# jhuldr/BrainFM

Measured on AMD Instinct MI355X. Metric: voxels/sec whole-volume multi-task inference, 256^3 tiled, higher is better.
Workload: dtype f16x3-split (fp32-grade); 1 GPU; 256^3 volume, reference tiling win160/stride80 -> 27 tiles, UNet3D f64 x6 levels, 9 heads (69 ch), fused tail + deformed atlas + on-device stitch of 17 keys; stitched_keys=17, mfma_passes=3, submission=hipGraph replay per tile shape, parallelism=tiles sharded over 1 rank(s), gather to rank 0, tiles_in_flight_per_gpu=2

## Files before the change

brainfm_amd/_lib.py:

```python
import ctypes as C
import os

_HERE = os.path.dirname(os.path.abspath(__file__))
LIB_PATH = os.path.join(_HERE, "libbrainfm_hip.so")

ERR = {0: "BFM_OK", -1: "BFM_E_ARG", -2: "BFM_E_SHAPE", -3: "BFM_E_WORKSPACE", -4: "BFM_E_LAUNCH"}

ROLE_PLAIN, ROLE_CT, ROLE_BIAS_LOG, ROLE_SEG, ROLE_DIST, ROLE_SR, ROLE_PATHOL = range(7)
(EW_EXP, EW_AFFINE, EW_CLAMP, EW_CLAMP_MIN, EW_GAMMA, EW_SIGMOID, EW_DIV, EW_NONZERO, EW_SUB_DIV, EW_GE,
 EW_NAN_TO_NUM) = range(11)
(EW_ADD, EW_MUL, EW_MUL_EXP, EW_AXPY_CLAMP0, EW_AXPY, EW_DIV2, EW_ZERO_WHERE_ZERO) = range(7)


class BfmError(RuntimeError):
    pass


class Upsample(C.Structure):
    _fields_ = [("d", C.c_int), ("h", C.c_int), ("w", C.c_int),
                ("mapD", C.c_void_p), ("mapH", C.c_void_p), ("mapW", C.c_void_p),
                ("repD", C.c_void_p), ("repH", C.c_void_p), ("repW", C.c_void_p)]


CLASS_STATS_BLOCKS = 1024
# ... 44 lines not shown
    _fields_ = [("V", C.c_void_p), ("n", C.c_int64)]


class GatherJob(C.Structure):
    _fields_ = [("src", C.c_void_p), ("out", C.c_void_p), ("mean", C.c_float), ("scale", C.c_float), ("pre", C.c_int),
                ("default_max", C.c_int), ("post_div", C.c_float), ("clamp", C.c_int), ("clamp_lo", C.c_float),
                ("clamp_hi", C.c_float), ("sign", C.c_float), ("want_minmax", C.c_int)]


_P = C.c_void_p
_I = C.c_int
_F = C.c_float
_L = C.c_int64
_Z = C.c_size_t
_UP = C.POINTER(Upsample)

SIGNATURES = {
    "bfm_version": (C.c_char_p, []),
    "bfm_gn_stats_workspace": (_Z, [_I, _I, _I, _I, _I, _UP]),
    "bfm_gn_stats": (_I, [_P, _I, _P, _I, _I, _I, _I, _UP, _P, _P, _I, _F, _P, _P, _P, _P, _Z, _P]),
    "bfm_pack_conv_weights_direct": (_I, [_P, _I, _I, _P, _P]),
    "bfm_pack_conv_weights_mfma_bytes": (_Z, [_I, _I]),
    "bfm_pack_conv_weights_mfma": (_I, [_P, _I, _I, _F, _P, C.POINTER(_I), _P]),
    "bfm_pack_conv_weights_mfma16_bytes": (_Z, [_I, _I]),
    "bfm_pack_conv_weights_mfma16": (_I, [_P, _I, _I, _F, _P, C.POINTER(_I), _P]),
    "bfm_conv3x3x3_direct": (_I, [_P, _I, _P, _I, _I, _I, _I, _UP, _P, _P, _P, _I, _F, _P, _P]),
    "bfm_pack_conv_weights_upfold_bytes": (C.c_size_t, [_I, _I, _I]),
    "bfm_pack_conv_weights_upfold": (_I, [_P, _I, _I, _I, _F, _I, _P, _P, _P]),
    "bfm_conv3x3x3_upfold": (_I, [_P, _I, _I, _I, _I, _P, _P, _P, _I, _P, _I, _I, _I, _P, _P]),
    "bfm_conv3x3x3_upfold_workspace": (_Z, [_I, _I, _I, _I, _I]),
    "bfm_conv3x3x3_upfold_ex": (_I, [_P, _I, _I, _I, _I, _P, _P, _P, _I, _P, _I, _I, _I, _P, _P, _Z, _P]),
    "bfm_conv3x3x3_upfold_batch_workspace": (_Z, [_I, _I, _I, _I, _I, _I]),
    "bfm_conv3x3x3_upfold_batch": (_I, [_P, _I, _I, _I, _I, _I, _P, _P, _P, _I, _P, _I, _I, _I, _P, _P, _Z, _I, _P]),
    "bfm_moment_rows_bytes": (_Z, [_I, _I]),
    "bfm_conv3x3x3_mfma_rows": (_I, [_I, _I, _I, _I, _I, C.POINTER(_I)]),
    "bfm_conv3x3x3_mfma_ex": (_I, [_P, _I, _P, _I, _I, _I, _I, _UP, _P, _P, _P, _I, _P, _I, _I, _F, _I,
                                   C.POINTER(_I), _P, _P, _Z, _P, _P]),
    "bfm_conv3x3x3_mfma_batch_workspace": (_Z, [_I, _I, _I, _I, _I, _I, _I]),
    "bfm_conv3x3x3_mfma_batch": (_I, [_P, _I, _P, _I, _I, _I, _I, _I, _UP, _P, _P, _P, _I, _P, _I, _I, _F, _I,
                                      C.POINTER(_I), _P, _P, _Z, _P, _I, _P]),
    "bfm_gn_stats_batch_workspace": (_Z, [_I, _I, _I, _I, _I, _I, _UP]),
    "bfm_gn_stats_batch": (_I, [_P, _I, _P, _I, _I, _I, _I, _I, _UP, _P, _P, _I, _F, _P, _P, _P, _P, _Z, _P]),
    "bfm_gn_stats_rows_batch": (_I, [_P, _I, _I, _P, _I, _I, C.c_double, _L, _I, _P, _P, _I, _F, _P, _P, _P, _P]),
    "bfm_conv3x3x3_stem_rows": (_I, [_I, _I, _I]),
    "bfm_conv3x3x3_stem_ex": (_I, [_P, _I, _I, _I, _P, _P, _P, _P, _I, _F, _P, _P, _P]),
    "bfm_conv3x3x3_stem_mc_ex": (_I, [_P, _I, _I, _I, _I, _P, _P, _P, _P, _I, _F, _P, _P, _P]),
    "bfm_gn_stats_rows_workspace": (_Z, [_I, _I, _I, _I]),
    "bfm_gn_stats_rows": (_I, [_P, _I, _I, _P, _I, _I, C.c_double, _L, _P, _P, _I, _F, _P, _P, _P, _P, _Z, _P, _P]),
    "bfm_gn_stats_rows_sliced": (_I, [_P, _I, _I, _I, _I, _P, _I, _I, _I, _I, C.c_double, _L, _P, _P, _I, _F, _P, _P, _P, _P, _Z,
                                      _P, _P]),
    "bfm_gn_stats_rows_train": (_I, [_P, _I, _I, _P, _I, _I, C.c_double, _L, _P, _P, _I, _F, _P, _P, _P, _P, _P, _P, _Z, _P, _P]),
    "bfm_crop3d": (_I, [_P, _I, _I, _I, _I, _I, _I, _I, _I, _I, _P, _P]),
    "bfm_pack_conv_weights_wino4_bytes": (_Z, [_I, _I, _I]),
    "bfm_pack_conv_weights_wino4": (_I, [_P, _I, _I, _F, _I, _P, C.POINTER(_I), _P]),
    "bfm_conv3x3x3_wino4_rows": (_I, [_I, _I, _I, _I]),
    "bfm_conv3x3x3_wino4_box": (_I, [_I, _I, _I, _I, _P]),
    "bfm_conv3x3x3_wino4_masked_workspace": (_Z, [_I, _I, _I, _I]),
    "bfm_conv3x3x3_wino4_uniform_scratch": (_Z, [_I]),
    "bfm_conv3x3x3_wino4_uniform": (_I, [_P, _I, _I, _I, _I, _P, _P, _P, _I, _P, _I, _I, _F, _I, _I, _P, _P, _P, _P, _P]),
    "bfm_conv3x3x3_wino4": (_I, [_P, _I, _I, _I, _I, _P, _P, _P, _I, _P, _I, _I, _F, _I, _I, _P, _P, _P]),
    "bfm_conv3x3x3_wino4_batch": (_I, [_P, _I, _I, _I, _I, _I, _P, _P, _P, _I, _P, _I, _I, _F, _I, _I, _P, _P, _I, _P]),
    "bfm_conv3x3x3_wino4_masked": (_I, [_P, _I, _I, _I, _I, _P, _P, _P, _I, _P, _I, _I, _F, _I, _I, _P, _P, _P, _Z, _P]),
    "bfm_permute_flip3d": (_I, [_P, _I, _I, _I, C.POINTER(_I), C.POINTER(_I), _P, _P]),
    "bfm_bbox_nonzero": (_I, [_P, _I, _I, _I, _F, _P, _P]),
    "bfm_mean_lastdim": (_I, [_P, _L, _I, _P, _P]),
    "bfm_pack_conv_weights_wino_bytes": (_Z, [_I, _I, _I]),
# ... 229 lines not shown
```

brainfm_amd/engine.py:

```python
import ctypes as C
import os
from collections import OrderedDict, namedtuple

import numpy as np
import torch

from . import _lib as L

LABELS_LEFT = [0, 1, 2, 3, 4, 7, 8, 9, 10, 14, 15, 17, 31, 34, 36, 38, 40, 42]
LABELS_FULL = [0, 11, 12, 13, 16, 31, 32, 33, 34, 35, 36, 37, 38, 39, 40, 41, 42, 43, 44, 46,
               1, 2, 3, 4, 5, 6, 7, 8, 9, 10, 14, 15, 17, 47, 49, 51, 53, 55,
               18, 19, 20, 21, 22, 23, 24, 25, 26, 27, 28, 29, 30, 48, 50, 52, 54, 56]


def features_per_level(f_maps, num_levels):
    return [f_maps * 2 ** k for k in range(num_levels)]


def nearest_index_map(n_in, n_out):
    scale = np.float32(n_in) / np.float32(n_out)
    idx = np.floor(np.arange(n_out, dtype=np.float32) * scale).astype(np.int64)
    return np.minimum(idx, n_in - 1).astype(np.int32)


_TUNE_CHOICES = {}

_Variant = namedtuple("_Variant", "layout pack_bytes pack rows box dense masked_workspace masked uniform_scratch uniform",
                      defaults=(None,) * 7)
_MFMA = _Variant("mfma", "bfm_pack_conv_weights_mfma_bytes", "bfm_pack_conv_weights_mfma")
_CONV_VARIANTS = (
    _MFMA,
    _MFMA,
    _Variant("mfma16", "bfm_pack_conv_weights_mfma16_bytes", "bfm_pack_conv_weights_mfma16"),
    _Variant("wino", "bfm_pack_conv_weights_wino_bytes", "bfm_pack_conv_weights_wino", "bfm_conv3x3x3_wino_rows",
             "bfm_conv3x3x3_wino_box", "bfm_conv3x3x3_wino_ex", "bfm_conv3x3x3_wino_masked_workspace",
             "bfm_conv3x3x3_wino_masked", "bfm_conv3x3x3_wino_uniform_scratch", "bfm_conv3x3x3_wino_uniform"),
    _Variant("wino4", "bfm_pack_conv_weights_wino4_bytes", "bfm_pack_conv_weights_wino4", "bfm_conv3x3x3_wino4_rows",
             "bfm_conv3x3x3_wino4_box", "bfm_conv3x3x3_wino4", "bfm_conv3x3x3_wino4_masked_workspace",
             "bfm_conv3x3x3_wino4_masked", "bfm_conv3x3x3_wino4_uniform_scratch", "bfm_conv3x3x3_wino4_uniform"),
)
_VARIANT_OF = {v.layout: ver for ver, v in enumerate(_CONV_VARIANTS)}

TUNE_FILE = os.environ.get("BFM_CONV_TUNE_FILE") or os.path.join(os.path.dirname(os.path.abspath(__file__)),
                                                                  "conv_tune_gfx950.json")
_TUNE_TABLE = None
_ARCH = {}


def _tune_key_str(key):
    cin, cout, dims, two, acc = key[:5]
    return ",".join(str(int(v)) for v in (cin, cout) + tuple(dims) + (two, acc) + tuple(key[5:]))


def _arch_of(dev_index):
    if dev_index not in _ARCH:
# ... 45 lines not shown

TRAIN_F43 = os.environ.get("BFM_TRAIN_F43", "1") != "0"


class _Layer:
    __slots__ = ("name", "cin", "cout", "groups", "gamma", "beta", "kind", "wpacked", "wexp", "w_raw", "packs", "skip",
                 "used")

    def touch(self, layout):
        u = getattr(self, "used", None)
        if u is None:
            u = self.used = set()
        u.add(layout)


HEAD_SLOPE = 0.2


class _HeadLayer(_Layer):
    __slots__ = ("bias",)


class UNetEngine:
    prof = None
    lane = 0
    weights_epoch = 0
    pack_count = 0
    _ws_lanes = None
    _variants = None
    _f23_ids = None
    _same_box_cache = None
    _uf_cache = None
    _deep_ok = None
    _head_layers = None
    _unit_bound = None
    _no_heads = None
    dense_last = False
    tape = None
    grad_sink = None
    prof_reps = 1
    use_upfold = False
    upfold_min = 250
    fuse_stats = False

    def __init__(self, state_dict, in_channels=1, f_maps=64, num_levels=6, num_groups=8, unit_feat=True,
                 device="cuda", passes=3, eps=1e-5, slope=0.01):
        self.lib = L.load()
        self.device = torch.device(device)
        if self.device.type != "cuda":
            raise L.BfmError("UNetEngine needs a HIP device; the product path has no CPU fallback")
        self.fm = features_per_level(f_maps, num_levels) if isinstance(f_maps, int) else list(f_maps)
        self.in_channels = in_channels
        self.num_groups = num_groups
        self.unit_feat = bool(unit_feat)
        self.passes = int(passes)
        self.eps = float(eps)
        self.slope = float(slope)
        self._up_cache = {}
        self._ws_lanes = {}
        self._ws_retired = []
        self.lane = 0
        self._gn_tickets = {ln: torch.zeros(16, dtype=torch.int32, device=self.device) for ln in range(4)}
        self._uf_tickets = {ln: torch.zeros(1, dtype=torch.int32, device=self.device) for ln in range(4)}
        self.gn_one_launch = os.environ.get("BFM_GN_ONE_LAUNCH", "1") != "0"
        self._plan_cache = {}
        self._tuned = set()
# ... 143 lines not shown
                    jobs.append((ly, layout, absmax(ly.w_raw[:, ly.skip.cin:])))
                elif layout == "direct":
                    jobs.append((ly, layout, None))
                else:
                    if wm is None:
                        wm = absmax(ly.w_raw)
                    jobs.append((ly, layout, wm))
            ly.used = set()
            ly.wpacked, ly.kind = None, None
            if ly.skip is not None:
                ly.skip.w_raw.copy_(ly.w_raw[:, :ly.skip.cin])
                visit(ly.skip)

        for pair in self.enc + self.dec + [hidden]:
            for ly in pair:
                visit(ly)
        host = slots[:nslot[0]].cpu().tolist() if nslot[0] else []
        for ly, layout, m in jobs:
            wmax = host[m] if m is not None else None
            if layout == "upfold":
                self._make_upfold_pack(ly, ly.skip.cin, ly.cin - ly.skip.cin, wmax)
            else:
                self._make_pack(ly, layout, wmax)

    def _upsample_desc(self, lo, hi):
        key = (tuple(lo), tuple(hi))
        if key not in self._up_cache:
            maps = [nearest_index_map(lo[a], hi[a]) for a in range(3)]
            reps = [np.bincount(maps[a], minlength=lo[a]).astype(np.int32) for a in range(3)]
            dev = [torch.from_numpy(m).to(self.device) for m in maps + reps]
            up = L.Upsample(lo[0], lo[1], lo[2], *[t.data_ptr() for t in dev])
            self._up_cache[key] = (up, dev)
        return self._up_cache[key][0]

    def _workspace(self, nbytes):
        nbytes = max(int(nbytes), 256)
        if self._ws_lanes is None:
            self._ws_lanes, self._ws_retired = {}, []
        ws = self._ws_lanes.get(self.lane)
        if ws is None or ws.numel() < nbytes:
            if ws is not None:
                self._ws_retired.append(ws)
            ws = self._ws_lanes[self.lane] = torch.empty(int(nbytes * 1.25) + 1024, dtype=torch.uint8, device=self.device)
        return ws

    def _uf_ticket(self):
        t = self._uf_tickets
        if self.lane not in t:
            t[self.lane] = torch.zeros(1, dtype=torch.int32, device=self.device)
        return t[self.lane]

    def _gn_ticket(self):
        t = self._gn_tickets
        if self.lane not in t:
            t[self.lane] = torch.zeros(16, dtype=torch.int32, device=self.device)
        return t[self.lane]

    def _plan(self, cin, cout, dims, two_src=False, accum=False):
        key = (cin, cout, tuple(dims), bool(two_src), bool(accum))
        if key not in self._plan_cache:
            cfg = (C.c_int * 8)()
            L.check(self.lib.bfm_conv3x3x3_mfma_plan(cin, cout, dims[0], dims[1], dims[2], cfg), "mfma_plan")
            if two_src and cfg[6] in (3, 4):
                cfg[6] = 0
            self._plan_cache[key] = cfg
        return self._plan_cache[key]
# ... 438 lines not shown
        if fused is not None and out is None and self.tape is None:
            return fused
        if out is None:
            out = torch.empty((D // 2, H // 2, W // 2, c), dtype=torch.float32, device=self.device)
        rows = self._rows_buf(c, 1, self.lib.bfm_maxpool2_rows, c, D, H, W)
        L.check(self.lib.bfm_maxpool2_ex(L.ptr(X), c, D, H, W, L.ptr(out), L.ptr(rows[0]) if rows is not None else None,
                                         L.stream_ptr()), "maxpool2")
        if rows is not None:
            out._bfm_rows = rows
        if self.tape is not None:
            self.tape.append(dict(pool_in=X, pool_dims=tuple(dims)))
        return out, (D // 2, H // 2, W // 2)

    def maxpool_batch(self, X, dims):
        S, (D, H, W), c = X.shape[0], dims, X.shape[-1]
        out = torch.empty((S, D // 2, H // 2, W // 2, c), dtype=torch.float32, device=self.device)
        if c % 4 or self.tape is not None:
            for s_ in range(S):
                self.maxpool(X[s_], dims, out=out[s_])
            return out
        rows = self._rows_buf(c, S, self.lib.bfm_maxpool2_batch_rows, c, D, H, W)
        L.check(self.lib.bfm_maxpool2_batch(L.ptr(X), c, S, D, H, W, L.ptr(out), L.ptr(rows[0]) if rows is not None else None,
                                            L.stream_ptr()), "maxpool2_batch")
        if rows is not None:
            out._bfm_rows = rows
        return out

    deep_from = int(os.environ.get("BFM_DEEP_FROM", "3"))
    deep_batch = os.environ.get("BFM_DEEP_BATCH", "1") != "0"
    DEEP_VERS = (0, 2)
    DEEP_VERS_1SRC = (0, 2, 4)
    deep_upfold = os.environ.get("BFM_DEEP_UPFOLD", "1") != "0"
    deep_upfold_min = int(os.environ.get("BFM_DEEP_UPFOLD_MIN", "100"))
    mask_skip = os.environ.get("BFM_MASK_SKIP", "1") != "0"
    uniform_skip = os.environ.get("BFM_UNIFORM_SKIP", "1") != "0"

    deep_vox = int(os.environ.get("BFM_DEEP_VOX", "16000"))

    def _region_ok(self, df):
        if self._deep_ok is None:
            self._deep_ok = {}
        cache = self._deep_ok
        if df not in cache:
            ndeep = len(self.enc) - 1 - df
            layers = [ly for pair in self.enc[df:] + self.dec[:ndeep] for ly in pair]
            cache[df] = all(ly.cin % 16 == 0 and ly.cout % 64 == 0 for ly in layers) and \
                self.enc[df - 1][1].cout % 16 == 0
        return cache[df]

    def has_deep_region(self):
        if not (self.deep_batch and self.tape is None and not self.force_direct and len(self.fm) > self.deep_from >= 1):
            return False
        return self._region_ok(self.deep_from)

    def region_start(self, dims):
        df = self.deep_from
        while df - 1 >= 2:
            lv = [v >> (df - 1) for v in dims]
            if min(lv) < 1 or lv[0] * lv[1] * lv[2] > self.deep_vox or not self._region_ok(df - 1):
                break
            df -= 1
        return df

    def _batch_stats(self, ly, A, ca, B, cb, S, dims, lo_dims, upp, scale, shift, bound):
        D, H, W = dims
        st = L.stream_ptr()
        ra = getattr(A, "_bfm_rows", None) if self.fuse_stats else None
        rb = getattr(B, "_bfm_rows", None) if (self.fuse_stats and B is not None) else None
        exact2 = B is None or tuple(dims) == tuple(2 * v for v in lo_dims)
        if ra is not None and ra[1] <= 128 and (B is None or (rb is not None and exact2 and rb[1] <= 128)):
            L.check(self.lib.bfm_gn_stats_rows_batch(L.ptr(ra[0]), ra[1], ca, L.ptr(rb[0]) if rb is not None else None,
                                                     rb[1] if rb is not None else 0, cb, 8.0, D * H * W, S,
                                                     L.ptr(ly.gamma), L.ptr(ly.beta), ly.groups, self.eps, L.ptr(scale),
                                                     L.ptr(shift), L.ptr(bound), st), "gn_stats_rows_batch " + ly.name)
            return
        need = self.lib.bfm_gn_stats_batch_workspace(ca, cb, S, D, H, W, upp)
        ws = self._workspace(need)
        L.check(self.lib.bfm_gn_stats_batch(L.ptr(A), ca, L.ptr(B), cb, S, D, H, W, upp, L.ptr(ly.gamma), L.ptr(ly.beta),
                                            ly.groups, self.eps, L.ptr(scale), L.ptr(shift), L.ptr(bound), L.ptr(ws),
                                            ws.numel(), st), "gn_stats_batch " + ly.name)

    def batch_conv(self, ly, A, dims, B=None, lo_dims=None, stats=None):
        S = A.shape[0]
        D, H, W = dims
        ca = A.shape[-1]
        cb = 0 if B is None else B.shape[-1]
        assert ca + cb == ly.cin, (ly.name, ca, cb, ly.cin)
        if not self._mfma_ok(ly, ca, cb):
            raise L.BfmError("%s: the batched levels need channel counts that are multiples of 16 / 64" % ly.name)
        up = self._upsample_desc(lo_dims, dims) if B is not None else None
        upp = C.byref(up) if up is not None else None
        if stats is None:
            scale = torch.empty((S, ly.cin), dtype=torch.float32, device=self.device)
            shift = torch.empty((S, ly.cin), dtype=torch.float32, device=self.device)
            bound = torch.empty((S, ly.groups), dtype=torch.float32, device=self.device)
            self._batch_stats(ly, A, ca, B, cb, S, dims, lo_dims, upp, scale, shift, bound)
        else:
            scale, shift, bound = stats
        if (B is not None and self.use_upfold and self.deep_upfold and tuple(dims) == tuple(2 * v for v in lo_dims)
                and lo_dims[0] * lo_dims[1] * lo_dims[2] >= self.deep_upfold_min):
            return self._batch_conv_upfold(ly, A, dims, B, lo_dims, scale, shift, bound)
        key = (ly.cin, ly.cout, tuple(dims), B is not None, False, 1)
        vers = self.DEEP_VERS if B is not None else self.DEEP_VERS_1SRC
        cfg = self._batch_plan(key, vers)
        out = torch.empty((S, D, H, W, ly.cout), dtype=torch.float32, device=self.device)
        if key not in self._tuned:
            cfg = self._autotune(ly, key, lambda c: self._batch_launch(ly, c, A[0:1], B[0:1] if B is not None else None, upp, dims,
                                                                       scale[0:1], shift[0:1], bound[0:1], out[0:1]),
                                 vers=vers)
        self._pack(ly, True, cfg[6])
        rows = self._rows_for(ly.cin, ly.cout, dims, cfg, S)
        nv = D * H * W
        lo = 0 if B is None else lo_dims[0] * lo_dims[1] * lo_dims[2]
        self._bracket(lambda: self._batch_launch(ly, cfg, A, B, upp, dims, scale, shift, bound, out, rows),
                      lambda: (2.0 * 27 * ly.cin * ly.cout * nv * S,
                               4.0 * (S * (nv * ca + lo * cb + nv * ly.cout) + 27 * ly.cin * ly.cout),
                               self._tag(ly) + ("x%d" % S), ly.cin, ly.cout, dims, cfg))
        if rows is not None:
            out._bfm_rows = rows
        return out

    def _batch_plan(self, key, vers):
        if key not in self._plan_cache:
            cfg = (C.c_int * 8)()
            L.check(self.lib.bfm_conv3x3x3_mfma_plan(key[0], key[1], key[2][0], key[2][1], key[2][2], cfg), "mfma_plan")
            if cfg[6] not in vers:
                cfg[6] = 0
            if key[4]:
                cfg[7] = 1
            self._plan_cache[key] = cfg
        return self._plan_cache[key]
# ... 24 lines not shown
        st = L.stream_ptr()
        sk = self._skip_layer(ly, ca)
        if "upfold" not in ly.packs:
            self._make_upfold_pack(ly, ca, cb)
        ly.touch("upfold")
        wup, wexp_up = ly.packs["upfold"]
        sc_a, sh_a = scale[:, :ca], shift[:, :ca]
        sc_b, sh_b = scale[:, ca:], shift[:, ca:]
        aff = ca + cb
        out = torch.empty((S, D, H, W, ly.cout), dtype=torch.float32, device=self.device)
        key = (ca, ly.cout, tuple(dims), False, True, 1)
        cfg = self._batch_plan(key, self.DEEP_VERS_1SRC)
        if key not in self._tuned:
            cfg = self._autotune(sk, key, lambda c: self._batch_launch(sk, c, A[0:1], None, None, dims, sc_a[0:1], sh_a[0:1],
                                                                       bound[0:1], out[0:1], None, aff),
                                 vers=self.DEEP_VERS_1SRC)
        self._pack(sk, True, cfg[6])
        nv = D * H * W
        lo = lo_dims[0] * lo_dims[1] * lo_dims[2]
        wsu = self.lib.bfm_conv3x3x3_upfold_batch_workspace(cb, S, lo_dims[0], lo_dims[1], lo_dims[2], ly.cout)

        def _launch_up():
            ws = self._workspace(wsu)
            L.check(self.lib.bfm_conv3x3x3_upfold_batch(L.ptr(B), cb, S, lo_dims[0], lo_dims[1], lo_dims[2], L.ptr(sc_b),
                                                        L.ptr(sh_b), L.ptr(bound), ly.groups, L.ptr(wup), wexp_up,
                                                        ly.cout, self.passes, L.ptr(out), L.ptr(ws) if wsu else None,
                                                        ws.numel() if wsu else 0, aff, st), "conv_upfold_batch " + ly.name)
        self._bracket(_launch_up, lambda: (2.0 * 27 * cb * ly.cout * nv * S, 4.0 * (S * (lo * cb + nv * ly.cout)),
                                           self._tag(ly) + "x%dup" % S, cb, ly.cout, dims, (0,) * 8))
        rows = self._rows_for(ca, ly.cout, dims, cfg, S)
        self._bracket(lambda: self._batch_launch(sk, cfg, A, None, None, dims, sc_a, sh_a, bound, out, rows, aff),
                      lambda: (2.0 * 27 * ca * ly.cout * nv * S, 4.0 * S * (nv * ca + 2 * nv * ly.cout),
                               self._tag(ly) + "x%dsk" % S, ca, ly.cout, dims, cfg))
        if rows is not None:
            out._bfm_rows = rows
        return out

    def deep_region(self, tops, df=None):
        S = len(tops)
        df = self.deep_from if df is None else df
        dims0 = tuple(tops[0][1])
        assert all(tuple(d) == dims0 for _, d in tops)
        c0 = tops[0][0].shape[-1]
        d = tuple(v // 2 for v in dims0)
        if min(dims0) < 2:
            raise L.BfmError("volume too small for %d pooling levels" % (len(self.enc) - 1))
        l1, l2 = self.enc[df]
        P = torch.empty((S,) + d + (c0,), dtype=torch.float32, device=self.device)
        scale = torch.empty((S, l1.cin), dtype=torch.float32, device=self.device)
        shift = torch.empty((S, l1.cin), dtype=torch.float32, device=self.device)
        bound = torch.empty((S, l1.groups), dtype=torch.float32, device=self.device)
        for s_, (x, dd) in enumerate(tops):
            ps, _ = self.maxpool(x, dd, out=P[s_])
            self._gn_stats(l1, ps, c0, None, 0, d, None, None, scale[s_], shift[s_], bound[s_], 0)
        x = self.batch_conv(l1, P, d, stats=(scale, shift, bound))
        x = self.batch_conv(l2, x, d)
        skips = [(x, d)]
        for i in range(df + 1, len(self.enc)):
            l1, l2 = self.enc[i]
            if min(d) < 2:
                raise L.BfmError("volume too small for %d pooling levels" % (len(self.enc) - 1))
            d2 = tuple(v // 2 for v in d)
            P = self.maxpool_batch(x, d)
            d = d2
            x = self.batch_conv(l1, P, d)
            x = self.batch_conv(l2, x, d)
# ... 328 lines not shown
```

include/brainfm_hip.h:

```cpp
#ifndef BRAINFM_HIP_H
#define BRAINFM_HIP_H

#include <stddef.h>
#include <stdint.h>

#ifdef __cplusplus
extern "C" {
#endif

typedef void* bfm_stream_t;

#define BFM_OK 0
#define BFM_E_ARG (-1)
#define BFM_E_SHAPE (-2)
#define BFM_E_WORKSPACE (-3)
#define BFM_E_LAUNCH (-4)

typedef struct {
    int d, h, w;
    const int32_t* mapD; const int32_t* mapH; const int32_t* mapW;
    const int32_t* repD; const int32_t* repH; const int32_t* repW;
} bfm_upsample_t;

const char* bfm_version(void);
// ... 119 lines not shown
                        int flags, float* out, void* moment_rows , bfm_stream_t stream);
int bfm_conv3x3x3_wino4_batch(const float* A, int CA, int S, int D, int H, int W, const float* scale, const float* shift,
                              const float* bound, int G, const void* wpacked, int wexp, int Cout, float slope, int passes,
                              int flags, float* out, void* moment_rows, int affine_stride, bfm_stream_t stream);
size_t bfm_conv3x3x3_wino4_masked_workspace(int D, int H, int W, int passes);
size_t bfm_conv3x3x3_wino4_uniform_scratch(int Cout);
int bfm_conv3x3x3_wino4_uniform(const float* A, int CA, int D, int H, int W, const float* scale, const float* shift,
                                const float* bound, int G, const void* wpacked, int wexp, int Cout, float slope, int passes,
                                int flags, float* out, void* moment_rows, const unsigned char* uniform_flags, void* scratch,
                                bfm_stream_t stream);
int bfm_conv3x3x3_wino4_masked(const float* A, int CA, int D, int H, int W, const float* scale, const float* shift,
                               const float* bound, int G, const void* wpacked, int wexp, int Cout, float slope, int passes,
                               int flags, float* out, const float* mask_image, void* workspace, size_t workspace_bytes,
                               bfm_stream_t stream);

size_t bfm_conv3x3x3_mfma_workspace(int Cin, int Cout, int D, int H, int W, int splitk);
int bfm_conv3x3x3_mfma_plan(int Cin, int Cout, int D, int H, int W, int* cfg_out );

size_t bfm_pack_conv_weights_upfold_bytes(int CB, int Cout, int passes);
int bfm_pack_conv_weights_upfold(const float* w_oidhw , int CA, int CB, int Cout,
                                 float wmax_abs_host, int passes, void* wpacked, int* wexp_host, bfm_stream_t stream);
int bfm_conv3x3x3_upfold(const float* B, int CB, int d, int h, int w, const float* scale_b, const float* shift_b,
                         const float* bound, int G, const void* wpacked, int wexp, int Cout, int passes, float* out,
                         bfm_stream_t stream);
size_t bfm_conv3x3x3_upfold_workspace(int CB, int d, int h, int w, int Cout);
int bfm_conv3x3x3_upfold_ex(const float* B, int CB, int d, int h, int w, const float* scale_b, const float* shift_b,
                            const float* bound, int G, const void* wpacked, int wexp, int Cout, int passes, float* out,
                            void* workspace, size_t workspace_bytes, bfm_stream_t stream);
size_t bfm_conv3x3x3_upfold_batch_workspace(int CB, int S, int d, int h, int w, int Cout);
int bfm_conv3x3x3_upfold_batch(const float* B, int CB, int S, int d, int h, int w, const float* scale_b,
                               const float* shift_b, const float* bound, int G, const void* wpacked, int wexp, int Cout,
                               int passes, float* out, void* workspace, size_t workspace_bytes, int affine_stride,
                               bfm_stream_t stream);

int bfm_conv3x3x3_mfma(const float* A, int CA, const float* B, int CB, int D, int H, int W,
                       const bfm_upsample_t* up, const float* scale, const float* shift, const float* bound,
                       int G, const void* wpacked, int wexp, int Cout, float slope, int passes,
                       const int* cfg , float* out, void* workspace,
                       size_t workspace_bytes, bfm_stream_t stream);

int bfm_maxpool2(const float* in, int C, int D, int H, int W, float* out, bfm_stream_t stream);

enum {
    BFM_ROLE_PLAIN = 0,
    BFM_ROLE_CT = 1,
    BFM_ROLE_BIAS_LOG = 2,
    BFM_ROLE_SEG = 3,
    BFM_ROLE_DIST = 4,
    BFM_ROLE_SR = 5,
    BFM_ROLE_PATHOL = 6
};
typedef struct {
    int n_out;
    int c_feat;
    const float* head_w;
    const float* head_b;
    const int32_t* roles;
    const int32_t* out_slot;
    int seg_first, n_seg;
    const int32_t* seg_lut;
    int n_dist;
    int dist_first;
    float max_dist;
    int unit_feat;
    int slot_high_res;
    int slot_fake_cortical;
// ... 350 lines not shown
```

Baseline: 204.5 million voxels/s.

## Add per-tap GEMM conv path for tiny deep-level volumes

Adds a new convolution path for very small spatial volumes (at most 64 low-res voxels). It packs the normalized activations once into f16 hi/lo splits, runs one MFMA GEMM per kernel tap (optionally split-K across slabs) to fill the CUs, then gathers and sums the 27 tap partials through a precomputed row table. That table also folds in nearest upsampling and applies the activation and moment stats. This is meant to fix the poor occupancy of the regular conv kernels on the deepest UNet levels, at the cost of extra workspace traffic for the partials and an additional launch.

```diff
diff --git a/brainfm_amd/_lib.py b/brainfm_amd/_lib.py
--- a/brainfm_amd/_lib.py
+++ b/brainfm_amd/_lib.py
@@ -100,6 +100,10 @@
     "bfm_conv3x3x3_upfold_ex": (_I, [_P, _I, _I, _I, _I, _P, _P, _P, _I, _P, _I, _I, _I, _P, _P, _Z, _P]),
     "bfm_conv3x3x3_upfold_batch_workspace": (_Z, [_I, _I, _I, _I, _I, _I]),
     "bfm_conv3x3x3_upfold_batch": (_I, [_P, _I, _I, _I, _I, _I, _P, _P, _P, _I, _P, _I, _I, _I, _P, _P, _Z, _I, _P]),
+    "bfm_conv3x3x3_tap_batch_workspace": (_Z, [_I, _I, _I, _I]),
+    "bfm_conv3x3x3_tap_batch": (_I, [_P, _I, _I, _I, _P, _P, _P, _I, _P, _I, _I, _I, _I, _I, _P, _Z, _I, _P]),
+    "bfm_tap_sum_rows": (_I, [_I, _I]),
+    "bfm_tap_sum_batch": (_I, [_P, _I, _I, _I, _I, _P, _I, _F, _I, _I, _P, _P, _P]),
     "bfm_moment_rows_bytes": (_Z, [_I, _I]),
     "bfm_conv3x3x3_mfma_rows": (_I, [_I, _I, _I, _I, _I, C.POINTER(_I)]),
     "bfm_conv3x3x3_mfma_ex": (_I, [_P, _I, _P, _I, _I, _I, _I, _UP, _P, _P, _P, _I, _P, _I, _I, _F, _I,
diff --git a/brainfm_amd/csrc/conv3d_tap.hip b/brainfm_amd/csrc/conv3d_tap.hip
--- /dev/null
+++ b/brainfm_amd/csrc/conv3d_tap.hip
@@ -0,0 +1,372 @@
+#include "conv_shared.h"
+
+namespace {
+
+typedef _Float16 half8 __attribute__((ext_vector_type(8)));
+typedef float floatx16 __attribute__((ext_vector_type(16)));
+
+constexpr int KC = 16;
+constexpr int TAP_MB = 4;
+constexpr int TAP_THREADS = 256;
+constexpr int TAP_LDS = 4 * TAP_MB * 2 * 16 * 64 * (int)sizeof(float);
+
+struct TapParams {
+    const float* X;
+    int Cin, S, n_lo, M, nmbt;
+    const float *scale, *shift;
+    int saff;
+    const float* bound;
+    int G;
+    const uint4* wp;
+    int wexp, Cout;
+    int kc0, kcn_pack;
+    int KCN, kc_per_slab, nslab;
+    uint4* apack;
+    float* rowdq;
+    float* P;
+};
+
+struct TapLayout {
+    int nmbt, nslab, per;
+    size_t off_apack, off_P, bytes;
+};
+
+void tap_split(int Cin, int Cout, int& nslab, int& per) {
+    const int KCN = Cin / KC;
+    const int wgs = (Cout / 64) * 27;
+    nslab = 1;
+    per = KCN;
+    if (wgs >= 256) return;
+    const int want = std::min(std::max(1, KCN / 3), bfm_cdiv(512, wgs));
+    if (want < 2) return;
+    per = bfm_cdiv(KCN, want);
+    nslab = bfm_cdiv(KCN, per);
+}
+
+bool tap_layout(int Cin, int Cout, int S, int n_lo, TapLayout& t) {
+    if (Cin <= 0 || Cout <= 0 || S <= 0 || n_lo <= 0 || Cin % KC || Cout % 64) return false;
+    const int64_t M = (int64_t)S * n_lo;
+    if (M > (1 << 20)) return false;
+    t.nmbt = (int)bfm_cdiv64(M, 32);
+    tap_split(Cin, Cout, t.nslab, t.per);
+    const size_t mpad = (size_t)t.nmbt * 32;
+    t.off_apack = (mpad * sizeof(float) + 255) / 256 * 256;
+    t.off_P = t.off_apack + (size_t)(Cin / KC) * t.nmbt * 2 * 64 * sizeof(uint4);
+    t.bytes = t.off_P + (size_t)27 * t.nslab * mpad * Cout * sizeof(float);
+    return true;
+}
+
+__global__ void __launch_bounds__(64) tap_prep(const TapParams p) {
+    const int lane = threadIdx.x;
+    const int kc = blockIdx.x, mb = blockIdx.y;
+    const int row = mb * 32 + (lane & 31);
+    const int k0 = kc * KC + 8 * (lane >> 5);
+    half8 hi, lo;
+#pragma unroll
+    for (int j = 0; j < 8; ++j) { hi[j] = (_Float16)0.f; lo[j] = (_Float16)0.f; }
+    float dq = 0.f;
+    if (row < p.M) {
+        const int smp = row / p.n_lo;
+        const float* pbound = p.bound + (size_t)smp * p.G;
+        float bmax = 0.f;
+        for (int g = 0; g < p.G; ++g) bmax = fmaxf(bmax, pbound[g]);
+        int aexp = 0;
+        if (bmax > 0.f && bmax < INFINITY) {
+            int ex;
+            (void)frexpf(bmax, &ex);
+            aexp = 14 - ex;
+            aexp = aexp > 60 ? 60 : (aexp < -60 ? -60 : aexp);
+        }
+        const float a_scale = ldexpf(1.0f, aexp);
+        dq = ldexpf(1.0f, -(aexp + p.wexp));
+        const float* x = p.X + (size_t)row * p.Cin + k0;
+        const float* sc = p.scale + (size_t)smp * p.saff + k0;
+        const float* sh = p.shift + (size_t)smp * p.saff + k0;
+#pragma unroll
+        for (int q = 0; q < 2; ++q) {
+            const float4 xv = *reinterpret_cast<const float4*>(x + 4 * q);
+            const float4 sv = *reinterpret_cast<const float4*>(sc + 4 * q);
+            const float4 hv = *reinterpret_cast<const float4*>(sh + 4 * q);
+            const float y[4] = {xv.x, xv.y, xv.z, xv.w};
+            const float s4[4] = {sv.x * a_scale, sv.y * a_scale, sv.z * a_scale, sv.w * a_scale};
+            const float h4[4] = {hv.x * a_scale, hv.y * a_scale, hv.z * a_scale, hv.w * a_scale};
+#pragma unroll
+            for (int i = 0; i < 4; ++i) {
+                const float t = fmaf(y[i], s4[i], h4[i]);
+                const _Float16 hh = (_Float16)t;
+                hi[4 * q + i] = hh;
+                lo[4 * q + i] = (_Float16)(t - (float)hh);
+            }
+        }
+    }
+    uint4* dst = p.apack + ((size_t)(kc * p.nmbt + mb) * 2) * 64 + lane;
+    dst[0] = __builtin_bit_cast(uint4, hi);
+    dst[64] = __builtin_bit_cast(uint4, lo);
+    if (kc == 0 && lane < 32) p.rowdq[row] = dq;
+}
+
+template <int NPASS>
+struct TapFrag {
+    uint4 w[4];
+    uint4 a[TAP_MB][2];
+};
+
+template <int NPASS>
+__global__ void __launch_bounds__(TAP_THREADS, 1) tap_gemm(const TapParams p) {
+    extern __shared__ __attribute__((aligned(16))) float tap_lds[];
+    const int tid = threadIdx.x;
+    const int lane = tid & 63;
+    const int wave = __builtin_amdgcn_readfirstlane(tid >> 6);
+    const int tap = blockIdx.x % 27;
+    const int r_ = blockIdx.x / 27;
+    const int slab = r_ % p.nslab, nt = r_ / p.nslab;
+    const int kcA = slab * p.kc_per_slab, kcB = min(p.KCN, kcA + p.kc_per_slab);
+    const uint4* const wb = p.wp + ((size_t)(nt * p.kcn_pack + p.kc0) * 27 + tap) * 256 + lane;
+    const int khalf = lane >> 5, l32 = lane & 31;
+    const size_t mpad = (size_t)p.nmbt * 32;
+    float* const Pt = p.P + ((size_t)(tap * p.nslab + slab) * mpad) * p.Cout + nt * 64 + khalf * 4;
+
+    for (int rg = 0; rg < p.nmbt; rg += TAP_MB) {
+        const int nmb = min(TAP_MB, p.nmbt - rg);
+        const uint4* const ab = p.apack + (size_t)rg * 128 + lane;
+        floatx16 acc[TAP_MB][2];
+#pragma unroll
+        for (int mb = 0; mb < TAP_MB; ++mb)
+#pragma unroll
+            for (int nb = 0; nb < 2; ++nb)
+#pragma unroll
+                for (int i = 0; i < 16; ++i) acc[mb][nb][i] = 0.f;
+
+        auto load = [&](int kc, TapFrag<NPASS>& f) __attribute__((always_inline)) {
+            if (kc >= kcB) return;
+            const uint4* w = wb + (size_t)kc * (27 * 256);
+            const uint4* a = ab + (size_t)kc * p.nmbt * 128;
+#pragma unroll
+            for (int nb = 0; nb < 2; ++nb) {
+                f.w[nb * 2] = w[nb * 128];
+                if constexpr (NPASS == 3) f.w[nb * 2 + 1] = w[nb * 128 + 64];
+            }
+#pragma unroll
+            for (int mb = 0; mb < TAP_MB; ++mb)
+                if (mb < nmb) {
+                    f.a[mb][0] = a[mb * 128];
+                    if constexpr (NPASS == 3) f.a[mb][1] = a[mb * 128 + 64];
+                }
+        };
+        auto compute = [&](const TapFrag<NPASS>& f) __attribute__((always_inline)) {
+#pragma unroll
+            for (int mb = 0; mb < TAP_MB; ++mb)
+                if (mb < nmb) {
+                    const half8 ahi = __builtin_bit_cast(half8, f.a[mb][0]);
+#pragma unroll
+                    for (int nb = 0; nb < 2; ++nb) {
+                        const half8 bhi = __builtin_bit_cast(half8, f.w[nb * 2]);
+                        if constexpr (NPASS == 3) {
+                            const half8 alo = __builtin_bit_cast(half8, f.a[mb][1]);
+                            const half8 blo = __builtin_bit_cast(half8, f.w[nb * 2 + 1]);
+                            acc[mb][nb] = __builtin_amdgcn_mfma_f32_32x32x16_f16(bhi, alo, acc[mb][nb], 0, 0, 0);
+                            acc[mb][nb] = __builtin_amdgcn_mfma_f32_32x32x16_f16(blo, ahi, acc[mb][nb], 0, 0, 0);
+                        }
+                        acc[mb][nb] = __builtin_amdgcn_mfma_f32_32x32x16_f16(bhi, ahi, acc[mb][nb], 0, 0, 0);
+                    }
+                }
+        };
+
+        TapFrag<NPASS> f0, f1, f2;
+        int kc = kcA + wave;
+        load(kc, f0);
+        load(kc + 4, f1);
+        for (; kc < kcB; kc += 12) {
+            load(kc + 8, f2);
+            __builtin_amdgcn_sched_barrier(0);
+            compute(f0);
+            if (kc + 4 < kcB) {
+                load(kc + 12, f0);
+                __builtin_amdgcn_sched_barrier(0);
+                compute(f1);
+            }
+            if (kc + 8 < kcB) {
+                load(kc + 16, f1);
+                __builtin_amdgcn_sched_barrier(0);
+                compute(f2);
+            }
+        }
+
+        float* const mine = tap_lds + (size_t)wave * (TAP_MB * 2 * 16 * 64) + lane;
+#pragma unroll
+        for (int mb = 0; mb < TAP_MB; ++mb)
+            if (mb < nmb) {
+#pragma unroll
+                for (int nb = 0; nb < 2; ++nb)
+#pragma unroll
+                    for (int i = 0; i < 16; ++i) mine[((mb * 2 + nb) * 16 + i) * 64] = acc[mb][nb][i];
+            }
+        __syncthreads();
+        if (wave < nmb) {
+            const int row = (rg + wave) * 32 + l32;
+            if (row < p.M) {
+                const float dq = p.rowdq[row];
+                float* const o = Pt + (size_t)row * p.Cout;
+                const float* const src = tap_lds + (size_t)(wave * 2) * 16 * 64 + lane;
+#pragma unroll
+                for (int nb = 0; nb < 2; ++nb)
+#pragma unroll
+                    for (int g = 0; g < 4; ++g) {
+                        float v[4];
+#pragma unroll
+                        for (int i = 0; i < 4; ++i) {
+                            const float* s = src + ((nb * 16) + 4 * g + i) * 64;
+                            float t = s[0];
+#pragma unroll
+                            for (int w = 1; w < 4; ++w) t += s[(size_t)w * (TAP_MB * 2 * 16 * 64)];
+                            v[i] = t * dq;
+                        }
+                        *reinterpret_cast<float4*>(o + nb * 32 + g * 8) = make_float4(v[0], v[1], v[2], v[3]);
+                    }
+            }
+        }
+        if (rg + TAP_MB < p.nmbt) __syncthreads();
+    }
+}
+
+__host__ __device__ inline int tap_cgb(int CG) { return (CG & 63) == 0 ? 64 : ((CG & 31) == 0 ? 32 : 16); }
+
+int tap_rows_vpb(int64_t nvox, int Cout) {
+    const int CG = Cout / 4, CGB = tap_cgb(CG), NV = 256 / CGB;
+    int64_t vpb = std::max<int64_t>((int64_t)NV * 4, bfm_cdiv64(nvox, 128));
+    vpb = bfm_cdiv64(vpb, NV) * NV;
+    return (int)std::min<int64_t>(vpb, 0x7fffffff);
+}
+
+__global__ void __launch_bounds__(256) tap_sum(const float* __restrict__ P, int nslab, int64_t mpad, int n_lo,
+                                               const int* __restrict__ table, int n_hi, int Cout, int vpb, int nrows,
+                                               float slope, int act, int accum, float* __restrict__ out,
+                                               double* __restrict__ rsum, double* __restrict__ rsq,
+                                               float* __restrict__ rmn, float* __restrict__ rmx) {
+    __shared__ float4 lsh[4][256];
+    const int CG = Cout >> 2;
+    const int CGB = tap_cgb(CG);
+    const int NV = 256 / CGB;
+    const int tid = threadIdx.x;
+    const int cgl = tid % CGB, vl = tid / CGB;
+    const int c4 = blockIdx.y * CGB + cgl;
+    const int smp = blockIdx.z, rb = blockIdx.x;
+    const int v0 = rb * vpb, v1 = min(n_hi, v0 + vpb);
+    const float4* P4 = reinterpret_cast<const float4*>(P) + (int64_t)smp * n_lo * CG + c4;
+    float4* o4 = reinterpret_cast<float4*>(out);
+    float4 fs = make_float4(0.f, 0.f, 0.f, 0.f), fq = fs;
+    float4 mn = make_float4(INFINITY, INFINITY, INFINITY, INFINITY), mx = make_float4(-INFINITY, -INFINITY, -INFINITY, -INFINITY);
+    for (int v = v0 + vl; v < v1; v += NV) {
+        const int* tb = table + (size_t)v * 27;
+        float4 a = make_float4(0.f, 0.f, 0.f, 0.f);
+#pragma unroll 9
+        for (int tap = 0; tap < 27; ++tap) {
+            const int r = tb[tap];
+            if (r < 0 || r >= n_lo) continue;
+            for (int k = 0; k < nslab; ++k) {
+                const float4 t = P4[((int64_t)(tap * nslab + k) * mpad + r) * CG];
+                a.x += t.x; a.y += t.y; a.z += t.z; a.w += t.w;
+            }
+        }
+        const int64_t i = ((int64_t)smp * n_hi + v) * CG + c4;
+        if (accum) {
+            const float4 t = o4[i];
+            a.x += t.x; a.y += t.y; a.z += t.z; a.w += t.w;
+        }
+        if (act) {
+            a.x = a.x >= 0.f ? a.x : a.x * slope; a.y = a.y >= 0.f ? a.y : a.y * slope;
+            a.z = a.z >= 0.f ? a.z : a.z * slope; a.w = a.w >= 0.f ? a.w : a.w * slope;
+        }
+        o4[i] = a;
+        fs.x += a.x; fs.y += a.y; fs.z += a.z; fs.w += a.w;
+        fq.x = fmaf(a.x, a.x, fq.x); fq.y = fmaf(a.y, a.y, fq.y); fq.z = fmaf(a.z, a.z, fq.z); fq.w = fmaf(a.w, a.w, fq.w);
+        mn.x = fminf(mn.x, a.x); mn.y = fminf(mn.y, a.y); mn.z = fminf(mn.z, a.z); mn.w = fminf(mn.w, a.w);
+        mx.x = fmaxf(mx.x, a.x); mx.y = fmaxf(mx.y, a.y); mx.z = fmaxf(mx.z, a.z); mx.w = fmaxf(mx.w, a.w);
+    }
+    if (!rsum) return;
+    lsh[0][tid] = fs; lsh[1][tid] = fq; lsh[2][tid] = mn; lsh[3][tid] = mx;
+    __syncthreads();
+    if (vl == 0) {
+        double S[4] = {0.0, 0.0, 0.0, 0.0}, Q[4] = {0.0, 0.0, 0.0, 0.0};
+        float MN[4] = {INFINITY, INFINITY, INFINITY, INFINITY}, MX[4] = {-INFINITY, -INFINITY, -INFINITY, -INFINITY};
+        for (int j = 0; j < NV; ++j) {
+            const float4 a = lsh[0][j * CGB + cgl], b = lsh[1][j * CGB + cgl], c = lsh[2][j * CGB + cgl], d = lsh[3][j * CGB + cgl];
+            S[0] += (double)a.x; S[1] += (double)a.y; S[2] += (double)a.z; S[3] += (double)a.w;
+            Q[0] += (double)b.x; Q[1] += (double)b.y; Q[2] += (double)b.z; Q[3] += (double)b.w;
+            MN[0] = fminf(MN[0], c.x); MN[1] = fminf(MN[1], c.y); MN[2] = fminf(MN[2], c.z); MN[3] = fminf(MN[3], c.w);
+            MX[0] = fmaxf(MX[0], d.x); MX[1] = fmaxf(MX[1], d.y); MX[2] = fmaxf(MX[2], d.z); MX[3] = fmaxf(MX[3], d.w);
+        }
+        const size_t o = ((size_t)smp * nrows + rb) * Cout + (size_t)c4 * 4;
+#pragma unroll
+        for (int k = 0; k < 4; ++k) { rsum[o + k] = S[k]; rsq[o + k] = Q[k]; rmn[o + k] = MN[k]; rmx[o + k] = MX[k]; }
+    }
+}
+
+}
+
+extern "C" size_t bfm_conv3x3x3_tap_batch_workspace(int Cin, int Cout, int S, int n_lo) {
+    TapLayout t;
+    return tap_layout(Cin, Cout, S, n_lo, t) ? t.bytes : 0;
+}
+
+extern "C" int bfm_conv3x3x3_tap_batch(const float* X, int Cin, int S, int n_lo, const float* scale, const float* shift,
+                                       const float* bound, int G, const void* wpacked, int wexp, int Cout, int kc_first,
+                                       int kc_pack, int passes, void* workspace, size_t workspace_bytes,
+                                       int affine_stride, bfm_stream_t stream) {
+    if (!X || !scale || !shift || !bound || G <= 0 || !wpacked || !workspace) return BFM_E_ARG;
+    if (passes != 1 && passes != 3) return BFM_E_ARG;
+    if (S <= 0 || S > 65535) return BFM_E_ARG;
+    TapLayout t;
+    if (!tap_layout(Cin, Cout, S, n_lo, t)) return BFM_E_SHAPE;
+    if (kc_first < 0 || kc_pack < kc_first + Cin / KC) return BFM_E_ARG;
+    if (affine_stride != 0 && (affine_stride < Cin || (affine_stride & 3))) return BFM_E_ARG;
+    if (workspace_bytes < t.bytes) return BFM_E_ARG;
+    if ((reinterpret_cast<uintptr_t>(X) & 15) || (reinterpret_cast<uintptr_t>(scale) & 15) ||
+        (reinterpret_cast<uintptr_t>(shift) & 15) || (reinterpret_cast<uintptr_t>(wpacked) & 15) ||
+        (reinterpret_cast<uintptr_t>(workspace) & 255))
+        return BFM_E_ARG;
+    const int64_t wgs = (int64_t)(Cout / 64) * 27 * t.nslab;
+    if (wgs > 0x7fffffff || t.nmbt > 65535) return BFM_E_SHAPE;
+    TapParams p{};
+    p.X = X; p.Cin = Cin; p.S = S; p.n_lo = n_lo; p.M = S * n_lo; p.nmbt = t.nmbt;
+    p.scale = scale; p.shift = shift; p.saff = affine_stride > 0 ? affine_stride : Cin;
+    p.bound = bound; p.G = G;
+    p.wp = static_cast<const uint4*>(wpacked);
+    p.wexp = wexp; p.Cout = Cout; p.kc0 = kc_first; p.kcn_pack = kc_pack;
+    p.KCN = Cin / KC; p.kc_per_slab = t.per; p.nslab = t.nslab;
+    char* ws = static_cast<char*>(workspace);
+    p.rowdq = reinterpret_cast<float*>(ws);
+    p.apack = reinterpret_cast<uint4*>(ws + t.off_apack);
+    p.P = reinterpret_cast<float*>(ws + t.off_P);
+    static bool attr = false;
+    if (const int rc = bfm_raise_lds_limit(attr, {bfm_kernel(&tap_gemm<3>), bfm_kernel(&tap_gemm<1>)}, TAP_LDS)) return rc;
+    hipLaunchKernelGGL(tap_prep, dim3((unsigned)p.KCN, (unsigned)t.nmbt), dim3(64), 0, bfm_s(stream), p);
+    bfm_launch_by_passes(passes, tap_gemm<3>, tap_gemm<1>, dim3((unsigned)wgs), dim3(TAP_THREADS), (size_t)TAP_LDS,
+                         bfm_s(stream), p);
+    return bfm_launch_status();
+}
+
+extern "C" int bfm_tap_sum_rows(int n_hi, int Cout) {
+    if (n_hi <= 0 || Cout <= 0 || Cout % 64) return 0;
+    return (int)bfm_cdiv64(n_hi, tap_rows_vpb(n_hi, Cout));
+}
+
+extern "C" int bfm_tap_sum_batch(const void* workspace, int Cin, int Cout, int S, int n_lo, const int* table, int n_hi,
+                                 float slope, int activation, int accumulate, float* out, void* moment_rows,
+                                 bfm_stream_t stream) {
+    if (!workspace || !table || !out || n_hi <= 0) return BFM_E_ARG;
+    if (S <= 0 || S > 65535) return BFM_E_ARG;
+    TapLayout t;
+    if (!tap_layout(Cin, Cout, S, n_lo, t)) return BFM_E_SHAPE;
+    if ((reinterpret_cast<uintptr_t>(workspace) & 255) || (reinterpret_cast<uintptr_t>(out) & 15)) return BFM_E_ARG;
+    const int vpb = tap_rows_vpb(n_hi, Cout);
+    const int nrows = (int)bfm_cdiv64(n_hi, vpb);
+    MomentRows mr;
+    if (moment_rows && !mr.carve(moment_rows, (size_t)S * nrows * Cout)) return BFM_E_ARG;
+    const int CG = Cout / 4, CGB = tap_cgb(CG);
+    const float* P = reinterpret_cast<const float*>(static_cast<const char*>(workspace) + t.off_P);
+    hipLaunchKernelGGL(tap_sum, dim3((unsigned)nrows, (unsigned)(CG / CGB), (unsigned)S), dim3(256), 0, bfm_s(stream), P,
+                       t.nslab, (int64_t)t.nmbt * 32, n_lo, table, n_hi, Cout, vpb, nrows, slope, activation ? 1 : 0,
+                       accumulate ? 1 : 0, out, mr.rsum, mr.rsq, mr.rmn, mr.rmx);
+    return bfm_launch_status();
+}
diff --git a/brainfm_amd/engine.py b/brainfm_amd/engine.py
--- a/brainfm_amd/engine.py
+++ b/brainfm_amd/engine.py
@@ -21,6 +21,21 @@
     scale = np.float32(n_in) / np.float32(n_out)
     idx = np.floor(np.arange(n_out, dtype=np.float32) * scale).astype(np.int64)
     return np.minimum(idx, n_in - 1).astype(np.int32)
+
+
+def tap_row_table(lo, hi):
+    maps = [nearest_index_map(lo[a], hi[a]).astype(np.int64) for a in range(3)]
+    z, y, x = np.meshgrid(*[np.arange(hi[a]) for a in range(3)], indexing="ij")
+    tab = np.full(tuple(hi) + (27,), -1, dtype=np.int32)
+    for kd in range(3):
+        for kh in range(3):
+            for kw in range(3):
+                zz, yy, xx = z + kd - 1, y + kh - 1, x + kw - 1
+                ok = (zz >= 0) & (zz < hi[0]) & (yy >= 0) & (yy < hi[1]) & (xx >= 0) & (xx < hi[2])
+                row = (maps[0][zz.clip(0, hi[0] - 1)] * lo[1] + maps[1][yy.clip(0, hi[1] - 1)]) * lo[2] \
+                    + maps[2][xx.clip(0, hi[2] - 1)]
+                tab[..., (kd * 3 + kh) * 3 + kw] = np.where(ok, row, -1)
+    return np.ascontiguousarray(tab.reshape(-1, 27))
 
 
 _TUNE_CHOICES = {}
@@ -132,6 +147,7 @@
     _same_box_cache = None
     _uf_cache = None
     _deep_ok = None
+    _tap_cache = None
     _head_layers = None
     _unit_bound = None
     _no_heads = None
@@ -341,6 +357,14 @@
             up = L.Upsample(lo[0], lo[1], lo[2], *[t.data_ptr() for t in dev])
             self._up_cache[key] = (up, dev)
         return self._up_cache[key][0]
+
+    def _tap_table(self, lo, hi):
+        key = (tuple(lo), tuple(hi))
+        if self._tap_cache is None:
+            self._tap_cache = {}
+        if key not in self._tap_cache:
+            self._tap_cache[key] = torch.from_numpy(tap_row_table(key[0], key[1])).to(self.device)
+        return self._tap_cache[key]
 
     def _workspace(self, nbytes):
         nbytes = max(int(nbytes), 256)
@@ -845,6 +869,8 @@
     DEEP_VERS_1SRC = (0, 2, 4)
     deep_upfold = os.environ.get("BFM_DEEP_UPFOLD", "1") != "0"
     deep_upfold_min = int(os.environ.get("BFM_DEEP_UPFOLD_MIN", "100"))
+    use_tap = os.environ.get("BFM_TAP", "1") != "0"
+    tap_max = 64
     mask_skip = os.environ.get("BFM_MASK_SKIP", "1") != "0"
     uniform_skip = os.environ.get("BFM_UNIFORM_SKIP", "1") != "0"
 
@@ -910,6 +936,8 @@
             self._batch_stats(ly, A, ca, B, cb, S, dims, lo_dims, upp, scale, shift, bound)
         else:
             scale, shift, bound = stats
+        if self.use_tap and (lo_dims[0] * lo_dims[1] * lo_dims[2] if B is not None else D * H * W) <= self.tap_max:
+            return self._batch_conv_tap(ly, A, dims, B, lo_dims, scale, shift, bound)
         if (B is not None and self.use_upfold and self.deep_upfold and tuple(dims) == tuple(2 * v for v in lo_dims)
                 and lo_dims[0] * lo_dims[1] * lo_dims[2] >= self.deep_upfold_min):
             return self._batch_conv_upfold(ly, A, dims, B, lo_dims, scale, shift, bound)
@@ -1000,6 +1028,55 @@
         self._bracket(lambda: self._batch_launch(sk, cfg, A, None, None, dims, sc_a, sh_a, bound, out, rows, aff),
                       lambda: (2.0 * 27 * ca * ly.cout * nv * S, 4.0 * S * (nv * ca + 2 * nv * ly.cout),
                                self._tag(ly) + "x%dsk" % S, ca, ly.cout, dims, cfg))
+        if rows is not None:
+            out._bfm_rows = rows
+        return out
+
+    def _batch_conv_tap(self, ly, A, dims, B, lo_dims, scale, shift, bound):
+        S = A.shape[0]
+        D, H, W = dims
+        nv = D * H * W
+        ca = A.shape[-1]
+        st = L.stream_ptr()
+        if "mfma" not in ly.packs:
+            self._make_pack(ly, "mfma")
+        ly.touch("mfma")
+        wp, wexp = ly.packs["mfma"]
+        out = torch.empty((S, D, H, W, ly.cout), dtype=torch.float32, device=self.device)
+        if B is None:
+            X, cx, n_lo, kc0, aff = A, ca, nv, 0, 0
+            sc_x, sh_x = scale, shift
+            tab = self._tap_table(dims, dims)
+            rows = self._rows_buf(ly.cout, S, self.lib.bfm_tap_sum_rows, nv, ly.cout)
+        else:
+            X, cx, n_lo, kc0, aff = B, B.shape[-1], lo_dims[0] * lo_dims[1] * lo_dims[2], ca // 16, ly.cin
+            sc_x, sh_x = scale[:, ca:], shift[:, ca:]
+            tab = self._tap_table(lo_dims, dims)
+            rows = None
+        wsb = self.lib.bfm_conv3x3x3_tap_batch_workspace(cx, ly.cout, S, n_lo)
+
+        def _launch_tap():
+            ws = self._workspace(wsb)
+            L.check(self.lib.bfm_conv3x3x3_tap_batch(L.ptr(X), cx, S, n_lo, L.ptr(sc_x), L.ptr(sh_x), L.ptr(bound), ly.groups,
+                                                     L.ptr(wp), wexp, ly.cout, kc0, ly.cin // 16, self.passes, L.ptr(ws),
+                                                     ws.numel(), aff, st), "conv_tap_batch " + ly.name)
+            L.check(self.lib.bfm_tap_sum_batch(L.ptr(ws), cx, ly.cout, S, n_lo, L.ptr(tab), nv, self.slope,
+                                               1 if B is None else 0, 0, L.ptr(out),
+                                               L.ptr(rows[0]) if rows is not None else None, st),
+                    "tap_sum_batch " + ly.name)
+        self._bracket(_launch_tap, lambda: (2.0 * 27 * cx * ly.cout * nv * S,
+                                            4.0 * (S * (n_lo * cx + nv * ly.cout) + 27 * cx * ly.cout),
+                                            self._tag(ly) + "x%dtap" % S, cx, ly.cout, dims, (0,) * 8))
+        if B is not None:
+            sk = self._skip_layer(ly, ca)
+            sc_a, sh_a = scale[:, :ca], shift[:, :ca]
+            key = (ca, ly.cout, tuple(dims), False, True, 1, "tap")
+            cfg = self._batch_plan(key, (0,))
+            self._pack(sk, True, 0)
+            rows = self._rows_for(ca, ly.cout, dims, cfg, S)
+            self._bracket(lambda: self._batch_launch(sk, cfg, A, None, None, dims, sc_a, sh_a, bound, out, rows, aff),
+                          lambda: (2.0 * 27 * ca * ly.cout * nv * S, 4.0 * S * (nv * ca + 2 * nv * ly.cout),
+                                   self._tag(ly) + "x%dsk" % S, ca, ly.cout, dims, cfg))
         if rows is not None:
             out._bfm_rows = rows
         return out
diff --git a/include/brainfm_hip.h b/include/brainfm_hip.h
--- a/include/brainfm_hip.h
+++ b/include/brainfm_hip.h
@@ -175,6 +175,15 @@
                                const float* shift_b, const float* bound, int G, const void* wpacked, int wexp, int Cout,
                                int passes, float* out, void* workspace, size_t workspace_bytes, int affine_stride,
                                bfm_stream_t stream);
+
+size_t bfm_conv3x3x3_tap_batch_workspace(int Cin, int Cout, int S, int n_lo);
+int bfm_conv3x3x3_tap_batch(const float* X, int Cin, int S, int n_lo, const float* scale, const float* shift,
+                            const float* bound, int G, const void* wpacked, int wexp, int Cout, int kc_first, int kc_pack,
+                            int passes, void* workspace, size_t workspace_bytes, int affine_stride, bfm_stream_t stream);
+int bfm_tap_sum_rows(int n_hi, int Cout);
+int bfm_tap_sum_batch(const void* workspace, int Cin, int Cout, int S, int n_lo, const int* table ,
+                      int n_hi, float slope, int activation, int accumulate, float* out, void* moment_rows ,
+                      bfm_stream_t stream);
 
 int bfm_conv3x3x3_mfma(const float* A, int CA, const float* B, int CB, int D, int H, int W,
                        const bfm_upsample_t* up, const float* scale, const float* shift, const float* bound,
```

Result: faster. 209.6 million voxels/s, median of 6 (+2.5%).
